# wgurecky/CORRLA_RS

Measured on AMD Instinct MI355X. Metric: RSVD GFLOP/s on 16k x 16k f32 rank-128, higher is better.
Workload: dtype f32

## Files before the change

### corrla_rs_amd/csrc/capi_impl.hpp

```cpp
#pragma once
#include <cstddef>
#include <cstdint>
#include <cstring>
#include <string>
#include <vector>

#include "../../include/corrla_rsvd.h"
#include "driver.hpp"

namespace corrla {

inline std::string& last_error_slot() {
  static thread_local std::string msg;
  return msg;
}

template <class F>
inline corrla_status guarded(F&& f) {
  try {
    f();
    return CORRLA_OK;
  } catch (const Error& e) {
    last_error_slot() = e.what();
    return (corrla_status)e.code;
// ... 158 lines not shown
}

template <class Dev, class T>
inline void finish_call(RsvdDriver<Dev, T>& drv, Dev& dev, Timings* tm_out, bool with_sketch_kernel_ms) {
  PhaseTimer fin;
  drv.phase(drv.tm.finalize_ms, fin);
  dev.phase_end();
  dev.end_call();
  dev.phase_resolve(&drv.tm.total_ms);
  drv.tm.n_collectives = dev.n_collectives;
  drv.tm.collective_bytes = dev.collective_bytes;
  if (with_sketch_kernel_ms) drv.tm.sketch_kernel_ms = dev.event_elapsed_ms(0, 1);
  if (tm_out) *tm_out = drv.tm;
}

template <class T>
struct RsvdCall {
  bool host_ptrs;
  int64_t m, rank, n_iter, n_oversamples;
  const corrla_opts* opts;
  T* u;
  int64_t ldu;
  T* s;
  T* vt;
  int64_t ldvt;
  Timings* tm_out;
  bool profile;
  bool sharded = false, sparse = false, fat = false, empty_shard = false;
  bool bf16 = false;
};
// ... 21 lines not shown
      },
      [&] {
        ta = stage();
        l = std::min<int64_t>(c.rank + c.n_oversamples, ta.nt);
        if (ro.omega && ro.omega_ld < ta.nt) throw Error(ST_EINVAL, "omega_ld < min(m, n)");
        u_in_place = !c.fat && !c.host_ptrs && !c.empty_shard;
        ut = u_in_place ? caller_skinny(c.u, ta.mt, k, c.ldu) : dev.template alloc_skinny<T>(ta.mt, k);
        vtall = dev.template alloc_skinny<T>(ta.nt, k);
        s_dev = dev.template alloc_scalar<T>((int)k);
      });
  RsvdDriver<Dev, T> drv(dev, c.profile);
  if (c.empty_shard) drv.m_local_override_ = 0;
  drv.random_svd_tall(ta, k, l, c.n_iter, ro, ut, s_dev, vtall, [&] {
    if (!c.fat) {
      if (!u_in_place && !c.empty_shard) dev.copy_out(ut, k, c.u, c.ldu, false, c.host_ptrs);
      dev.copy_out(vtall, k, c.vt, c.ldvt, true, c.host_ptrs);
    } else {
      dev.copy_out(vtall, k, c.u, c.ldu, false, c.host_ptrs);
      if (!c.empty_shard) dev.copy_out(ut, k, c.vt, c.ldvt, true, c.host_ptrs);
    }
    dev.copy_values_out(s_dev, k, c.s, c.host_ptrs);
  });
  finish_call(drv, dev, c.tm_out, true);
}

template <class Dev, class T>
inline void rsvd_entry(Dev& dev, bool host_ptrs, bool sharded, const T* a, int64_t m, int64_t n, int64_t rs, int64_t cs,
                       int64_t rank, int64_t n_iter, int64_t n_oversamples, const corrla_opts* opts, T* u, int64_t ldu,
                       T* s, T* vt, int64_t ldvt, Timings* tm_out, bool profile) {
  const bool shard_cols = sharded && opts && (opts->flags & CORRLA_SHARD_COLS) != 0;
  const bool empty_shard = sharded && m >= 0 && n >= 0 && (shard_cols ? (n == 0 && m >= 1) : (m == 0 && n >= 1));
  const int64_t short_side = shard_cols ? m : n;
  RsvdCall<T> c{host_ptrs, m, rank, n_iter, n_oversamples, opts, u, ldu, s, vt, ldvt, tm_out, profile};
  c.sharded = sharded;
  c.fat = sharded ? shard_cols : m < n;
  c.empty_shard = empty_shard;
// ... 104 lines not shown
    } else {
      dev.center_rows_cols(ta.mem.p, ta.mem.rows, ta.mem.cols, ta.mem.ld, mu.p, data_cols_along_mem_cols, cbuf, ldp);
    }
    tc.mem.p = cbuf;
    tc.mem.ld = ldp;
    tc.mem.cols_readable = ldp;
  }
  const int64_t k = c.rank;
  const int64_t l = std::min<int64_t>(c.rank + c.n_oversamples, tc.nt);
  if (ro.omega && ro.omega_ld < tc.nt) throw Error(ST_EINVAL, "omega_ld < min(m, n)");
  Skinny<T> ut = dev.template alloc_skinny<T>(tc.mt, k);
  Skinny<T> vtall = dev.template alloc_skinny<T>(tc.nt, k);
  T* s_dev = dev.template alloc_scalar<T>((int)k);
  if (tc.inv_sd_short || tc.inv_sd_tall) drv.set_scale_workspace(dev.template alloc_skinny<T>(c.n, l));
  drv.random_svd_tall(tc, k, l, c.n_iter, ro, ut, s_dev, vtall, [&] {
    dev.copy_out(fat ? ut : vtall, k, c.comps, c.ldc, true, c.host_ptrs);
    dev.copy_values_out(s_dev, k, c.s, c.host_ptrs);
    dev.copy_values_out(mu.p, c.n, c.means, c.host_ptrs);
    if (scales_out) dev.copy_values_out(sd.p, c.n, scales_out, c.host_ptrs);
  });
  finish_call(drv, dev, c.tm_out, false);
}

template <class Dev, class T>
inline void pca_entry(Dev& dev, bool host_ptrs, const T* x, int64_t m, int64_t n, int64_t rs, int64_t cs, int64_t rank,
                      int64_t n_iter, int64_t n_oversamples, const corrla_opts* opts, T* means, T* s, T* comps,
                      int64_t ldc, Timings* tm_out, bool profile, bool sharded = false) {
  PcaCall<T> c{host_ptrs, m, n, rank, n_iter, n_oversamples, opts, means, s, comps, ldc, tm_out, profile};
  c.sharded = sharded;
  pca_body(
      dev, c,
      [&] {
// ... 249 lines not shown
```

### corrla_rs_amd/csrc/core_svd_stage.hpp

```cpp
#pragma once
#include "core_svd_plan.hpp"
#include "hip_backend.hpp"

namespace corrla {

template <class T>
struct CoreSvdCall {
  const Skinny<T>& c;
  int64_t l, k;
  Skinny<T>&m1, &m2;
  T* s_dev;
  void* conv_status;
};

namespace core_svd_stage {

template <class T>
using RingEs = std::integer_sequence<int, 8, 12, 16, sizeof(T) == 4 ? 20 : 18>;
constexpr int kMaxNc = 9;

template <class T>
inline void set_lds_limits() {
  for_each_of(RingEs<T>{}, [](auto e) { lds_limit((const void*)k::jacobi_ring_w_kernel<T, decltype(e)::value, 8>, k::kLdsMaxBytes); });
  lds_limit((const void*)k::jacobi_block_round_kernel<T>, k::kLdsMaxBytes);
// ... 146 lines not shown
  kn.jmc_np = env_int("CORRLA_JMC_NP", kn.jmc_np);
  kn.jmc_sweeps_f32 = env_int("CORRLA_JMC_SWEEPS", kn.jmc_sweeps_f32);
  kn.jmc_sweeps_f64 = env_int("CORRLA_JMC_SWEEPS", kn.jmc_sweeps_f64);
  kn.jmc_force_v = env_int("CORRLA_JMC_FORCE_V", 0) != 0;
  kn.strict = env_int("CORRLA_JACOBI_STRICT", 0) != 0;
  kn.block_sweeps = env_int("CORRLA_JACOBI_SWEEPS", kn.block_sweeps);
  kn.ring_sweeps = env_int("CORRLA_JACOBI_SWEEPS", kn.ring_sweeps);
  kn.block_inner = env_int("CORRLA_JACOBI_INNER", kn.block_inner);
  return kn;
}

}

template <class T>
void HipDev::small_svd(const Skinny<T>& c, int64_t l, int64_t k, Skinny<T>& m1, Skinny<T>& m2, T* s_dev, void* conv_status) {
  if (conv_status) memset_zero(conv_status, sizeof(k::CholStatus));
  const CoreSvdCall<T> a{c, l, k, m1, m2, s_dev, conv_status};
  const CoreSvdPlan plan = core_svd_plan((int)sizeof(T), l, k, core_svd_stage::knobs_from_env(), svd_state_, conv_status != nullptr);
  switch (plan.family) {
    case CoreSvd::kMultiWg:
      core_svd_stage::multi_wg(*this, a, plan);
      return;
    case CoreSvd::kHost:
      small_svd_host(*this, c, l, k, m1, m2, s_dev);
      return;
    case CoreSvd::kBlock:
      core_svd_stage::finite_check(*this, a);
      core_svd_stage::block(*this, a, plan);
      return;
    case CoreSvd::kRing:
      core_svd_stage::finite_check(*this, a);
// ... 7 lines not shown
```

### corrla_rs_amd/csrc/driver.hpp

```cpp
#pragma once
#include <cstdio>
#include <chrono>
#include <cmath>
#include <cstdint>
#include <cstring>
#include <limits>
#include <stdexcept>
#include <string>
#include <functional>
#include <type_traits>
#include <vector>

#include "gemm_plan.hpp"
#include "small_linalg.hpp"

namespace corrla {

struct Error : std::runtime_error {
  int code;
  Error(int c, const std::string& m) : std::runtime_error(m), code(c) {}
};
enum { ST_OK = 0, ST_EINVAL = 1, ST_ENOMEM = 2, ST_EHIP = 3, ST_ECOMM = 4, ST_ENUMERIC = 5, ST_ENODEV = 6 };

inline int64_t round_up(int64_t x, int64_t a) { return (x + a - 1) / a * a; }
// ... 43 lines not shown

template <class D, class = void>
struct dev_has_spmm : std::false_type {};
template <class D>
struct dev_has_spmm<D, std::void_t<decltype(D::kHasSpmm)>> : std::true_type {};

template <class D, class = void>
struct dev_has_bf16in : std::false_type {};
template <class D>
struct dev_has_bf16in<D, std::void_t<decltype(D::kHasBf16In)>> : std::true_type {};

template <class D, class = void>
struct dev_has_colvar : std::false_type {};
template <class D>
struct dev_has_colvar<D, std::void_t<decltype(D::kHasColVar)>> : std::true_type {};

template <class T>
struct TallA {
  Big<T> mem;
  bool row_major = true;
  int64_t mt = 0, nt = 0;
  const T* mu_short = nullptr;
  const T* mu_tall = nullptr;
  const T* inv_sd_short = nullptr;
  const T* inv_sd_tall = nullptr;
  bool sparse = false;
  CsrView<T> csr, csr_t;
  bool bf16 = false;
  Big<uint16_t> mem16;
};
// ... 91 lines not shown
    else if (a.bf16)
      bf16_times(!a.row_major, a.mem16, x, y, scale_dev);
    else if (mixed_planes_ && dev.template mixed_fits<T>(!a.row_major, a.mem, x, y))
      dev.gemm_mixed(!a.row_major, a.mem, x, y, scale_dev, mixed_planes_), ++tm.n_mixed_products;
    else if (a.row_major)
      dev.gemm_nn(a.mem, x, y, scale_dev);
    else
      dev.gemm_tn(a.mem, x, y, scale_dev);
    if (a.mu_short || a.mu_tall) {
      T* v = dev.template alloc_scalar<T>((int)x.cols_alloc);
      dev.weighted_colsum(x, a.nt, a.mu_short, v);
      dev.rank1_sub(y, a.mt, a.mu_tall, v, scale_dev);
    }
    if (a.inv_sd_tall) scale_output(y, a.mt, a.inv_sd_tall);
  }
  void at_times(const TallA<T>& a, const Skinny<T>& y_in, Skinny<T>& z, const T* scale_dev, bool sharded) {
    const Skinny<T> y = a.inv_sd_tall ? scaled_input(y_in, a.mt, a.inv_sd_tall) : y_in;
    if (a.sparse)
      sparse_times(a.csr_t, y, z, scale_dev);
    else if (a.bf16)
      bf16_times(a.row_major, a.mem16, y, z, scale_dev);
    else if (mixed_planes_ && dev.template mixed_fits<T>(a.row_major, a.mem, y, z))
      dev.gemm_mixed(a.row_major, a.mem, y, z, scale_dev, mixed_planes_), ++tm.n_mixed_products;
    else if (a.row_major)
      dev.gemm_tn(a.mem, y, z, scale_dev);
    else
      dev.gemm_nn(a.mem, y, z, scale_dev);
    if (a.mu_short || a.mu_tall) {
      T* v = dev.template alloc_scalar<T>((int)y.cols_alloc);
      dev.weighted_colsum(y, a.mt, a.mu_tall, v);
      dev.rank1_sub(z, a.nt, a.mu_short, v, scale_dev);
// ... 436 lines not shown
      }
      a_times(a, z, y, kNone);
      i0 = nf;
    } else {
      dev.event_mark(0);
      a_times(a, om, y, kNone);
      dev.event_mark(1);
      phase(tm.sketch_ms, pt);
    }
    for (int64_t i = i0; i < n_iter; ++i) {
      if (i > 2) {
        phase(tm.power_ms, pt);
        orthonormalize(y, y2, o.sharded, true);
        phase(tm.qr_ms, pt);
      }
      at_times(a, y, z, kNone, o.sharded);
      dev.inv_norm(z, ss_dev, inv_dev);
      dev.scale_inplace(z, inv_dev);
      a_times(a, z, y, kNone);
    }
    phase(tm.power_ms, pt);
    int64_t r = orthonormalize(y, y2, o.sharded);
    phase(tm.qr_ms, pt);
    return r;
  }

  void random_svd_tall(const TallA<T>& a, int64_t k, int64_t l, int64_t n_iter, const RunOpts& o, Skinny<T>& u_tall,
                       T* s_dev, Skinny<T>& v_tall, const std::function<void()>& emit = {}) {
    qr_householder = o.qr_householder;
    m_local_ = m_local_override_ >= 0 ? m_local_override_ : a.mt;
    m_global_ = -1;
    hh_short_shards_ = -1;
    const bool hh = qr_householder;
    if (!hh && (dev.template device_chol_fits<T>(l) || dev.template device_chol_blocked_fits<T>(l))) {
      const Timings saved = tm;
      const auto mark = dev.arena_mark();
      bool on_device = true;
      for (int attempt = 0; attempt < 5 && on_device; ++attempt) {
        if (attempt > 0) dev.arena_rewind(mark);
// ... 100 lines not shown
    }
    return need[p.npass - 1] != 0 ? Verdict::kMorePasses : Verdict::kClean;
  }
  Verdict judge_core_svd(const Pending& p, const StatusRecord& r) {
    debug_record(p.record, "core SVD", r);
    if (r.fail == 0) dev.svd_sweeps_used((int)r.dev_i);
    if (r.fail == 1) return Verdict::kMoreSweeps;
    if (r.fail == 4) return Verdict::kNeedV;
    return r.fail == 0 ? Verdict::kClean : Verdict::kRepeatOnHost;
  }

  void random_svd_tall_body(const TallA<T>& a, int64_t k, int64_t l, int64_t n_iter, const RunOpts& o, Skinny<T>& u_tall,
                            T* s_dev, Skinny<T>& v_tall) {
    PhaseTimer total;
    const bool hh_tmp = qr_householder;
    Skinny<T> q = dev.template alloc_skinny_out<T>(a.mt, l);
    Skinny<T> q2 = hh_tmp ? dev.template alloc_skinny<T>(a.mt, l) : dev.template alloc_skinny_out<T>(a.mt, l);
    power_iter(a, l, n_iter, o, q, q2);
    PhaseTimer pt;
    Skinny<T> bt = dev.template alloc_skinny<T>(a.nt, l);
    mixed_planes_ = o.mixed_project ? o.mixed_planes : 0;
    at_times(a, q, bt, kNone, o.sharded);
    mixed_planes_ = 0;
    phase(tm.project_ms, pt);
    Skinny<T> qb = dev.template alloc_skinny<T>(a.nt, l);
    Skinny<T> qb2 = dev.template alloc_skinny<T>(a.nt, l);
    dev.copy_skinny(bt, qb);
    orthonormalize(qb, qb2, false);
    phase(tm.qr_ms, pt);
    Skinny<T> ct = dev.template alloc_skinny<T>(l, l);
    dev.gemm_nn(as_rowmajor_transposed(bt, l), qb, ct, kNone);
    if (o.poison_core) dev.poison_entry(ct, l / 2, l / 3, o.poison_core);
    Skinny<T> m1 = dev.template alloc_skinny<T>(l, k);
    Skinny<T> m2 = dev.template alloc_skinny<T>(l, k);
    void* svd_st = nullptr;
    if (att_.defer && att_.st_used + 1 <= att_.st_slots) {
      svd_st = status_record(att_.st_used);
      att_.pending.push_back(Pending::core_svd(att_.st_used));
      att_.st_used += 1;
    }
    dev.small_svd(ct, l, k, m2, m1, s_dev, svd_st);
    if (att_.defer) {
// ... 94 lines not shown
```

### corrla_rs_amd/csrc/hip_backend.hpp

```cpp
#pragma once
#include <hip/hip_runtime.h>
#include <rccl/rccl.h>

#include <cmath>
#include <cstdio>
#include <cstdlib>
#include <cstring>
#include <limits>
#include <random>
#include <string>
#include <type_traits>
#include <utility>
#include <vector>

#include "core_svd_plan.hpp"
#include "driver.hpp"
#include "hip_kernels.hpp"
#include "tsqr_kernels.hpp"
#include "jacobi_mc_kernels.hpp"
#include "ata_kernels.hpp"
#include "tall_kernels.hpp"
#include "mixed_kernels.hpp"
#include "bf16in_kernels.hpp"
#include "grad_kernels.hpp"
// ... 161 lines not shown
      *nranks_out = 0;
      return;
    }
    CORRLA_NCCL(ncclCommUserRank(comm, rank_out));
    CORRLA_NCCL(ncclCommCount(comm, nranks_out));
  }

  void begin_call() {
    CORRLA_HIP(hipSetDevice(device));
    events_set_[0] = events_set_[1] = events_set_[2] = false;
    n_collectives = 0;
    collective_bytes = 0;
    marks_.clear();
    ev_used_ = 0;
    phase_mark(nullptr);
    for (auto& c : chunks_) c.used = 0;
    sp_scratch_ = nullptr;
    sp_scratch_bytes_ = 0;
    for (auto& c : zchunks_) {
      c.zeroed = std::min<size_t>(c.used, (size_t)256 << 20);
      c.used = 0;
      if (c.zeroed) CORRLA_HIP(hipMemsetAsync(c.p, 0, c.zeroed, stream));
    }
  }
  void end_call() { sync(); }
  void sync() { CORRLA_HIP(hipStreamSynchronize(stream)); }

  void* alloc_bytes(size_t bytes) {
    bytes = (bytes + 255) / 256 * 256;
    if (bytes == 0) bytes = 256;
// ... 61 lines not shown
    s.cols = cols;
    s.ld = round_up(std::max<int64_t>(rows, 1), kLdPad);
    s.cols_alloc = col_blocking(cols).cols_alloc;
    const size_t bytes = (size_t)s.ld * (size_t)s.cols_alloc * sizeof(T);
    if (bytes < ((size_t)4 << 20)) {
      s.p = (T*)alloc_zeroed(bytes);
      return s;
    }
    s.p = (T*)alloc_bytes(bytes);
    if (s.ld > rows)
      CORRLA_HIP(hipMemset2DAsync(s.p + rows, (size_t)s.ld * sizeof(T), 0, (size_t)(s.ld - rows) * sizeof(T), (size_t)s.cols_alloc,
                                  stream));
    if (s.cols_alloc > cols) memset_zero(s.p + cols * s.ld, (size_t)(s.cols_alloc - cols) * s.ld * sizeof(T));
    return s;
  }
  double* alloc_f64(int n) {
    return (double*)alloc_zeroed(sizeof(double) * n);
  }
  template <class T>
  T* alloc_scalar(int n) {
    return (T*)alloc_zeroed(sizeof(T) * n);
  }

  void h2d_2d(void* dst, int64_t dpitch_e, const void* src, int64_t spitch_e, int64_t width_e, int64_t rows, size_t esz) {
    CORRLA_HIP(hipMemcpy2DAsync(dst, (size_t)dpitch_e * esz, src, (size_t)spitch_e * esz, (size_t)width_e * esz,
                                (size_t)rows, hipMemcpyHostToDevice, stream));
    sync();
  }
  template <class T>
  void h2d_2d(T* dst, int64_t dpitch_e, const T* src, int64_t spitch_e, int64_t width_e, int64_t rows) {
    h2d_2d((void*)dst, dpitch_e, (const void*)src, spitch_e, width_e, rows, sizeof(T));
  }

  template <class T>
  void gemm_nn(const Big<T>& r, const Skinny<T>& x, Skinny<T>& out, const T* scale_dev) {
    if (x.rows != r.cols) throw Error(ST_EINVAL, "gemm_nn: inner dimensions differ");
    launch_gemm<T>(false, r, x, out, scale_dev);
  }
  template <class T>
  void gemm_tn(const Big<T>& r, const Skinny<T>& x, Skinny<T>& out, const T* scale_dev) {
    if (x.rows != r.rows) throw Error(ST_EINVAL, "gemm_tn: inner dimensions differ");
    launch_gemm<T>(true, r, x, out, scale_dev);
  }

  static constexpr bool kHasSpmm = true;
  template <class T>
  void csr_plan(CsrView<T>& v, bool check_idx) {
    k::CsrCounts* cnt = (k::CsrCounts*)alloc_zeroed(sizeof(k::CsrCounts));
    const int64_t top = std::max(v.rows, v.nnz);
    const unsigned blocks = (unsigned)std::max<int64_t>(1, std::min<int64_t>((top + 255) / 256, (int64_t)num_cus * 16));
    hipLaunchKernelGGL(k::csr_validate_kernel, dim3(blocks), dim3(256), 0, stream, v.rp, v.ci, v.rows, v.cols, v.nnz, check_idx ? 1 : 0, cnt);
    CORRLA_HIP(hipGetLastError());
    k::CsrCounts h;
    read_bytes(cnt, sizeof(h), &h);
    if (h.bad) {
      std::string why;
      if (h.bad & 1) why += " row_ptr[0] != 0;";
// ... 585 lines not shown
  void householder_thin_q(Skinny<T>& y, Skinny<T>& tmp) {
    HhState<T> h = householder_up(y, tmp);
    householder_down(h, y, tmp);
  }
  template <class T>
  int householder_max_width() const {
    int w = 1;
    while (householder_fits<T>(w + 1)) ++w;
    return w;
  }
  int rank() const { return comm_rank; }

  template <class T>
  void small_svd(const Skinny<T>& c, int64_t l, int64_t k, Skinny<T>& m1, Skinny<T>& m2, T* s_dev, void* conv_status);
  template <class T>
  void copy_out(const Skinny<T>& src, int64_t ncols, T* dst, int64_t ldd, bool transpose, bool to_host) {
    const int64_t rows = src.rows;
    if (!to_host) {
      launch_copy_out(src.p, src.ld, rows, ncols, dst, ldd, transpose);
      return;
    }
    if (!transpose) {
      CORRLA_HIP(hipMemcpy2DAsync(dst, (size_t)ldd * sizeof(T), src.p, (size_t)src.ld * sizeof(T),
                                  (size_t)rows * sizeof(T), (size_t)ncols, hipMemcpyDeviceToHost, stream));
    } else {
      T* tmp = (T*)alloc_bytes((size_t)rows * ncols * sizeof(T));
      launch_copy_out(src.p, src.ld, rows, ncols, tmp, ncols, true);
      CORRLA_HIP(hipMemcpy2DAsync(dst, (size_t)ldd * sizeof(T), tmp, (size_t)ncols * sizeof(T),
                                  (size_t)ncols * sizeof(T), (size_t)rows, hipMemcpyDeviceToHost, stream));
    }
    sync();
  }
  template <class T>
  void pack_strided(const T* src, int64_t rows, int64_t cols, int64_t rs, int64_t cs, T* dst, int64_t ldd) {
    const int64_t tiles_c = (cols + 31) / 32, tiles_r = (rows + 31) / 32;
    if (tiles_c * tiles_r > 0x7fffffff) throw Error(ST_EINVAL, "problem too large for the launch grid");
    dim3 grid((unsigned)(tiles_c * tiles_r));
    hipLaunchKernelGGL((k::pack_strided_kernel<T>), grid, dim3(256), 0, stream, src, rows, cols, rs, cs, dst, ldd, tiles_c);
    CORRLA_HIP(hipGetLastError());
  }

  template <class T>
  void weighted_colsum(const Skinny<T>& x, int64_t rows, const T* w, T* v) {
    const int ncols = (int)x.cols_alloc;
    const int nblk = (int)std::max<int64_t>(1, std::min<int64_t>(64, (rows + 4095) / 4096));
    double* partial = (double*)alloc_bytes(sizeof(double) * (size_t)nblk * (size_t)ncols);
// ... 226 lines not shown
  hipEvent_t events_[3] = {nullptr, nullptr, nullptr};
  bool events_set_[3] = {false, false, false};
  struct PhaseMark {
    hipEvent_t ev;
    double* slot;
  };
  std::vector<hipEvent_t> ev_pool_;
  size_t ev_used_ = 0;
  std::vector<PhaseMark> marks_;
  static constexpr size_t kPinnedBytes = (size_t)8 << 20;
  int gemm_debug_flags_ = 0;
  GemmKnobs gemm_knobs_;
  uint64_t entropy_ = 0, calls_ = 0, calls_sharded_ = 0;
  bool no_device_chol_ = false;
  const int* run_if_ = nullptr;
  bool phase_events_ = true;
  bool robust_qr_ = true;
  int robust_passes_ = 2;
  CoreSvdState svd_state_;

  static void check_grid(const dim3& g) {
    if (g.y > 65535u || g.z > 65535u) throw Error(ST_EINVAL, "problem too large for the launch grid");
  }

  static void set_lds_limits() {
    constexpr size_t kMax = k::kLdsMaxBytes;
    set_lds_limits_typed<float>();
    set_lds_limits_typed<double>();
    core_svd_stage::set_lds_limits<float>();
    core_svd_stage::set_lds_limits<double>();
// ... 104 lines not shown
  void launch_general(bool tn, const GemmPlan& p, dim3 grid, dim3 block, int lds, const k::GemmArgs<T>& a) {
    with_nt<2>(p.mw, [&](auto mw) {
      with_nt<8, 4>(p.nw, [&](auto nw) {
        constexpr int MW = decltype(mw)::value, NW = decltype(nw)::value;
        if constexpr (NW == 4 || (NW == 8 && MW == 1 && std::is_same<T, double>::value)) {
          if (tn)
            hipLaunchKernelGGL((k::gemm_tn_kernel<T, MW, NT, NW>), grid, block, lds, stream, a);
          else
            hipLaunchKernelGGL((k::gemm_nn_kernel<T, MW, NT, false, NW>), grid, block, lds, stream, a);
        }
      });
    });
  }

  template <class T>
  void launch_gemm(bool tn, const Big<T>& r, const Skinny<T>& x, Skinny<T>& out, const T* scale_dev) {
    const GemmPlan p = plan_gemm(tn, r, x, out, 0);
    const GemmLaunch& L0 = p.launch[0];
    T* slab = p.reduce.kind != SlabReduce::none ? (T*)alloc_bytes(p.slab_bytes) : nullptr;
    if (p.family == GemmFamily::tall_apply) {
      const k::TallApplyArgs<T> g{r.p, r.cols, r.ld, (int)r.rows, x.p, x.ld, (int)x.cols, out.p, out.ld, (int)p.out_cols,
                                  scale_dev, p.vec_store, run_if_};
      with_nt<sizeof(T) == 4 ? 6 : 4>(L0.nt, [&](auto kt) {
        constexpr int K = decltype(kt)::value;
        hipLaunchKernelGGL((k::tall_apply_kernel<T, K, K>), dim3(L0.grid[0]), dim3(p.block), L0.lds, stream, g);
      });
    } else if (p.family == GemmFamily::tall_gram) {
      const k::TallGramArgs<T> g{x.p, r.cols, x.ld, (int)out.rows, slab, p.slab_stride, out.ld, p.rows_per_group,
                                 (const T*)zero_page_, run_if_};
      with_nt<sizeof(T) == 4 ? 6 : 4>(L0.nt, [&](auto nct) {
        hipLaunchKernelGGL((k::tall_gram_kernel<T, decltype(nct)::value>), dim3(L0.grid[0]), dim3(p.block), L0.lds, stream, g);
// ... 7 lines not shown
                       p.vec_store, p.rotate, p.outer_blocks, 0};
      for (int i = 0; i < p.nlaunch; ++i) {
        const GemmLaunch& L = p.launch[i];
        const dim3 grid(L.grid[0], L.grid[1], L.grid[2]), block(p.block);
        a.col_base = L.col_base;
        a.xcd_remap = L.xcd_remap;
        if (p.family == GemmFamily::gram_alias)
          with_nt<8>(L.nt, [&](auto nt) {
            hipLaunchKernelGGL((k::gemm_nn_kernel<T, 2, decltype(nt)::value, true>), grid, block, L.lds, stream, a);
          });
        else
          with_nt<kMaxColTiles>(L.nt, [&](auto nt) { launch_general<T, decltype(nt)::value>(tn, p, grid, block, L.lds, a); });
      }
    }
    CORRLA_HIP(hipGetLastError());
    slab_reduce<T>(p.reduce, slab, p.slab_stride, out.p, out.ld, scale_dev, run_if_);
  }

  template <class T>
  void launch_copy_out(const T* src, int64_t lds_, int64_t rows, int64_t cols, T* dst, int64_t ldd, bool transpose) {
    const int64_t tiles_c = (cols + 31) / 32, tiles_r = (rows + 31) / 32;
    if (tiles_c * tiles_r > 0x7fffffff) throw Error(ST_EINVAL, "problem too large for the launch grid");
    dim3 grid((unsigned)(tiles_c * tiles_r));
    hipLaunchKernelGGL((k::copy_out_kernel<T>), grid, dim3(256), 0, stream, src, lds_, rows, cols, dst, ldd,
                       transpose ? 1 : 0, tiles_c);
    CORRLA_HIP(hipGetLastError());
  }
};

}
```

### corrla_rs_amd/csrc/hip_kernels.hpp

```cpp
#pragma once
#include <hip/hip_runtime.h>

#include <limits>
#include <stdint.h>

#include <type_traits>

#include "gemm_plan.hpp"

namespace corrla {
namespace k {

typedef float f32x4 __attribute__((ext_vector_type(4)));
typedef double f64x4 __attribute__((ext_vector_type(4)));
typedef double f64x2 __attribute__((ext_vector_type(2)));

#ifndef CORRLA_F32_BIG_IS_A
#define CORRLA_F32_BIG_IS_A true
#endif
template <class T>
struct MT;
template <>
struct MT<float> {
  typedef f32x4 acc_t;
// ... 672 lines not shown
    const double v = (double)y[i];
    s += v * v;
  }
  for (int off = 32; off > 0; off >>= 1) s += __shfl_down(s, off, 64);
  __shared__ double ws[4];
  if ((threadIdx.x & 63) == 0) ws[threadIdx.x >> 6] = s;
  __syncthreads();
  if (threadIdx.x == 0) partial[blockIdx.x] = ws[0] + ws[1] + ws[2] + ws[3];
}
__global__ void sum_partials_kernel(const double* partial, int n, double* out) {
  double s = 0.0;
  for (int i = threadIdx.x; i < n; i += 64) s += partial[i];
  for (int off = 32; off > 0; off >>= 1) s += __shfl_down(s, off, 64);
  if (threadIdx.x == 0) *out = s;
}
template <class T>
__global__ void sum_partials_rsqrt_kernel(const double* partial, int n, double* ss_out, T* inv_out) {
  double s = 0.0;
  for (int i = threadIdx.x; i < n; i += 64) s += partial[i];
  for (int off = 32; off > 0; off >>= 1) s += __shfl_down(s, off, 64);
  if (threadIdx.x == 0) {
    *ss_out = s;
    *inv_out = (T)(s > 0.0 ? 1.0 / sqrt(s) : 0.0);
  }
}
template <class T>
__global__ void rsqrt_scalar_kernel(const double* ss, T* out) {
  const double v = *ss;
  *out = (T)(v > 0.0 ? 1.0 / sqrt(v) : 0.0);
}
template <class T>
__global__ void sub_kernel(T* y, const T* __restrict__ p, int64_t n) {
  for (int64_t i = (int64_t)blockIdx.x * blockDim.x + threadIdx.x; i < n; i += (int64_t)gridDim.x * blockDim.x) y[i] -= p[i];
}
template <class T>
__global__ void scale_kernel(T* y, int64_t n, const T* scale) {
  const T sc = *scale;
  for (int64_t i = (int64_t)blockIdx.x * blockDim.x + threadIdx.x; i < n; i += (int64_t)gridDim.x * blockDim.x)
// ... 1191 lines not shown
  const int tx = threadIdx.x & 31, ty = threadIdx.x >> 5;
  const bool col_fast = cs <= rs;
  for (int q = ty; q < 32; q += 8) {
    const int64_t r = col_fast ? r0 + q : r0 + tx;
    const int64_t c = col_fast ? c0 + tx : c0 + q;
    if (r < rows && c < cols) tile[r - r0][c - c0] = src[r * rs + c * cs];
  }
  __syncthreads();
  for (int q = ty; q < 32; q += 8) {
    const int64_t r = r0 + q, c = c0 + tx;
    if (r < rows && c < cols) dst[r * ldd + c] = tile[q][tx];
  }
}
template <class T>
__global__ void copy_out_kernel(const T* src, int64_t lds_, int64_t rows, int64_t cols, T* dst, int64_t ldd, int transpose,
                                int64_t tiles_c) {
  __shared__ T tile[32][33];
  const int64_t r0 = ((int64_t)blockIdx.x / tiles_c) * 32, c0 = ((int64_t)blockIdx.x % tiles_c) * 32;
  const int tx = threadIdx.x & 31, ty = threadIdx.x >> 5;
  if (!transpose) {
    for (int q = ty; q < 32; q += 8) {
      const int64_t r = r0 + tx, c = c0 + q;
      if (r < rows && c < cols) dst[c * ldd + r] = src[c * lds_ + r];
    }
    return;
  }
  for (int q = ty; q < 32; q += 8) {
    const int64_t r = r0 + tx, c = c0 + q;
    if (r < rows && c < cols) tile[q][tx] = src[c * lds_ + r];
  }
  __syncthreads();
  for (int q = ty; q < 32; q += 8) {
// ... 8 lines not shown
```

Measured before the change: 93540.

## Fuse RSVD tail ops into slab reduce, copy-out and padding kernels

Adds several tail fusions. The split-K slab reduction now also writes a second copy of the output (replacing a separate copy_skinny) and emits per-block sum-of-squares partials, so normalisation takes one scale kernel instead of a norm-then-scale pair. Singular values ride along in the copy-out kernel, the conv-status memset is skipped, and the two output Q buffers are padded by one zeroing kernel. The aim is fewer small kernel launches and fewer passes over the skinny matrices, at the cost of extra code paths gated on plan family and the CORRLA_TAIL_UNFUSED env var.

```diff
diff --git a/corrla_rs_amd/csrc/capi_impl.hpp b/corrla_rs_amd/csrc/capi_impl.hpp
--- a/corrla_rs_amd/csrc/capi_impl.hpp
+++ b/corrla_rs_amd/csrc/capi_impl.hpp
@@ -196,6 +196,17 @@
   if (tm_out) *tm_out = drv.tm;
 }
 
+template <class Dev, class T>
+inline void copy_out_with_s(Dev& dev, const Skinny<T>& src, int64_t k, T* dst, int64_t ldd, bool transpose, bool host_ptrs,
+                            const T* s_dev, T* s_out) {
+  if constexpr (dev_has_tail_fusions<Dev>::value) {
+    dev.copy_out_with_values(src, k, dst, ldd, transpose, host_ptrs, s_dev, s_out, k);
+  } else {
+    dev.copy_out(src, k, dst, ldd, transpose, host_ptrs);
+    dev.copy_values_out(s_dev, k, s_out, host_ptrs);
+  }
+}
+
 template <class T>
 struct RsvdCall {
   bool host_ptrs;
@@ -247,12 +258,11 @@
   drv.random_svd_tall(ta, k, l, c.n_iter, ro, ut, s_dev, vtall, [&] {
     if (!c.fat) {
       if (!u_in_place && !c.empty_shard) dev.copy_out(ut, k, c.u, c.ldu, false, c.host_ptrs);
-      dev.copy_out(vtall, k, c.vt, c.ldvt, true, c.host_ptrs);
+      copy_out_with_s(dev, vtall, k, c.vt, c.ldvt, true, c.host_ptrs, s_dev, c.s);
     } else {
-      dev.copy_out(vtall, k, c.u, c.ldu, false, c.host_ptrs);
       if (!c.empty_shard) dev.copy_out(ut, k, c.vt, c.ldvt, true, c.host_ptrs);
+      copy_out_with_s(dev, vtall, k, c.u, c.ldu, false, c.host_ptrs, s_dev, c.s);
     }
-    dev.copy_values_out(s_dev, k, c.s, c.host_ptrs);
   });
   finish_call(drv, dev, c.tm_out, true);
 }
@@ -387,8 +397,7 @@
   T* s_dev = dev.template alloc_scalar<T>((int)k);
   if (tc.inv_sd_short || tc.inv_sd_tall) drv.set_scale_workspace(dev.template alloc_skinny<T>(c.n, l));
   drv.random_svd_tall(tc, k, l, c.n_iter, ro, ut, s_dev, vtall, [&] {
-    dev.copy_out(fat ? ut : vtall, k, c.comps, c.ldc, true, c.host_ptrs);
-    dev.copy_values_out(s_dev, k, c.s, c.host_ptrs);
+    copy_out_with_s(dev, fat ? ut : vtall, k, c.comps, c.ldc, true, c.host_ptrs, s_dev, c.s);
     dev.copy_values_out(mu.p, c.n, c.means, c.host_ptrs);
     if (scales_out) dev.copy_values_out(sd.p, c.n, scales_out, c.host_ptrs);
   });
diff --git a/corrla_rs_amd/csrc/core_svd_stage.hpp b/corrla_rs_amd/csrc/core_svd_stage.hpp
--- a/corrla_rs_amd/csrc/core_svd_stage.hpp
+++ b/corrla_rs_amd/csrc/core_svd_stage.hpp
@@ -184,7 +184,7 @@
 
 template <class T>
 void HipDev::small_svd(const Skinny<T>& c, int64_t l, int64_t k, Skinny<T>& m1, Skinny<T>& m2, T* s_dev, void* conv_status) {
-  if (conv_status) memset_zero(conv_status, sizeof(k::CholStatus));
+  if (conv_status && tail_unfused_) memset_zero(conv_status, sizeof(k::CholStatus));
   const CoreSvdCall<T> a{c, l, k, m1, m2, s_dev, conv_status};
   const CoreSvdPlan plan = core_svd_plan((int)sizeof(T), l, k, core_svd_stage::knobs_from_env(), svd_state_, conv_status != nullptr);
   switch (plan.family) {
diff --git a/corrla_rs_amd/csrc/driver.hpp b/corrla_rs_amd/csrc/driver.hpp
--- a/corrla_rs_amd/csrc/driver.hpp
+++ b/corrla_rs_amd/csrc/driver.hpp
@@ -81,6 +81,28 @@
 struct dev_has_colvar : std::false_type {};
 template <class D>
 struct dev_has_colvar<D, std::void_t<decltype(D::kHasColVar)>> : std::true_type {};
+
+template <class D, class = void>
+struct dev_has_tail_fusions : std::false_type {};
+template <class D>
+struct dev_has_tail_fusions<D, std::void_t<decltype(D::kHasTailFusions)>> : std::true_type {};
+
+template <class T>
+struct ProductTaps {
+  T* copy_to = nullptr;
+  bool want_sumsq = false;
+  bool copied = false;
+  const double* partial = nullptr;
+  int nparts = 0;
+};
+struct TapContext {
+  bool tail_fused = false;
+  bool sparse = false, bf16 = false, centred = false, standardised = false, sharded = false;
+  int mixed_planes = 0;
+};
+inline bool product_taps_apply(const TapContext& c) {
+  return c.tail_fused && !c.sparse && !c.bf16 && c.mixed_planes == 0 && !c.centred && !c.standardised && !c.sharded;
+}
 
 template <class T>
 struct TallA {
@@ -202,7 +224,26 @@
     }
     if (a.inv_sd_tall) scale_output(y, a.mt, a.inv_sd_tall);
   }
-  void at_times(const TallA<T>& a, const Skinny<T>& y_in, Skinny<T>& z, const T* scale_dev, bool sharded) {
+  bool tail_fused() const {
+    if constexpr (dev_has_tail_fusions<Dev>::value)
+      return dev.tail_fused();
+    else
+      return false;
+  }
+  bool taps_apply(const TallA<T>& a, bool sharded) const {
+    TapContext c;
+    c.tail_fused = tail_fused();
+    c.sparse = a.sparse, c.bf16 = a.bf16, c.mixed_planes = mixed_planes_, c.sharded = sharded;
+    c.centred = a.mu_short || a.mu_tall, c.standardised = a.inv_sd_short || a.inv_sd_tall;
+    return product_taps_apply(c);
+  }
+  void at_times(const TallA<T>& a, const Skinny<T>& y_in, Skinny<T>& z, const T* scale_dev, bool sharded, ProductTaps<T>* taps = nullptr) {
+    if (taps && taps_apply(a, sharded)) {
+      if constexpr (dev_has_tail_fusions<Dev>::value) {
+        dev.gemm_tapped(a.row_major, a.mem, y_in, z, scale_dev, *taps);
+        return;
+      }
+    }
     const Skinny<T> y = a.inv_sd_tall ? scaled_input(y_in, a.mt, a.inv_sd_tall) : y_in;
     if (a.sparse)
       sparse_times(a.csr_t, y, z, scale_dev);
@@ -669,15 +710,29 @@
         orthonormalize(y, y2, o.sharded, true);
         phase(tm.qr_ms, pt);
       }
-      at_times(a, y, z, kNone, o.sharded);
-      dev.inv_norm(z, ss_dev, inv_dev);
-      dev.scale_inplace(z, inv_dev);
+      ProductTaps<T> taps;
+      taps.want_sumsq = true;
+      at_times(a, y, z, kNone, o.sharded, &taps);
+      if (!normalize_from_taps(z, taps, ss_dev, inv_dev)) {
+        dev.inv_norm(z, ss_dev, inv_dev);
+        dev.scale_inplace(z, inv_dev);
+      }
       a_times(a, z, y, kNone);
     }
     phase(tm.power_ms, pt);
     int64_t r = orthonormalize(y, y2, o.sharded);
     phase(tm.qr_ms, pt);
     return r;
+  }
+
+  bool normalize_from_taps(Skinny<T>& z, const ProductTaps<T>& taps, double* ss_dev, T* inv_dev) {
+    if constexpr (dev_has_tail_fusions<Dev>::value) {
+      if (taps.nparts > 0) {
+        dev.scale_by_partials(z, taps, ss_dev, inv_dev);
+        return true;
+      }
+    }
+    return false;
   }
 
   void random_svd_tall(const TallA<T>& a, int64_t k, int64_t l, int64_t n_iter, const RunOpts& o, Skinny<T>& u_tall,
@@ -808,18 +863,26 @@
                             T* s_dev, Skinny<T>& v_tall) {
     PhaseTimer total;
     const bool hh_tmp = qr_householder;
-    Skinny<T> q = dev.template alloc_skinny_out<T>(a.mt, l);
-    Skinny<T> q2 = hh_tmp ? dev.template alloc_skinny<T>(a.mt, l) : dev.template alloc_skinny_out<T>(a.mt, l);
+    Skinny<T> q, q2;
+    if constexpr (dev_has_tail_fusions<Dev>::value) {
+      if (!hh_tmp) dev.template alloc_skinny_out2<T>(a.mt, l, q, q2);
+    }
+    if (!q.p) {
+      q = dev.template alloc_skinny_out<T>(a.mt, l);
+      q2 = hh_tmp ? dev.template alloc_skinny<T>(a.mt, l) : dev.template alloc_skinny_out<T>(a.mt, l);
+    }
     power_iter(a, l, n_iter, o, q, q2);
     PhaseTimer pt;
     Skinny<T> bt = dev.template alloc_skinny<T>(a.nt, l);
+    Skinny<T> qb = dev.template alloc_skinny<T>(a.nt, l);
+    ProductTaps<T> bt_taps;
+    bt_taps.copy_to = qb.p;
     mixed_planes_ = o.mixed_project ? o.mixed_planes : 0;
-    at_times(a, q, bt, kNone, o.sharded);
+    at_times(a, q, bt, kNone, o.sharded, &bt_taps);
     mixed_planes_ = 0;
     phase(tm.project_ms, pt);
-    Skinny<T> qb = dev.template alloc_skinny<T>(a.nt, l);
     Skinny<T> qb2 = dev.template alloc_skinny<T>(a.nt, l);
-    dev.copy_skinny(bt, qb);
+    if (!bt_taps.copied) dev.copy_skinny(bt, qb);
     orthonormalize(qb, qb2, false);
     phase(tm.qr_ms, pt);
     Skinny<T> ct = dev.template alloc_skinny<T>(l, l);
diff --git a/corrla_rs_amd/csrc/hip_backend.hpp b/corrla_rs_amd/csrc/hip_backend.hpp
--- a/corrla_rs_amd/csrc/hip_backend.hpp
+++ b/corrla_rs_amd/csrc/hip_backend.hpp
@@ -199,6 +199,7 @@
     marks_.clear();
     ev_used_ = 0;
     phase_mark(nullptr);
+    tail_unfused_ = env_int("CORRLA_TAIL_UNFUSED", 0) != 0;
     for (auto& c : chunks_) c.used = 0;
     sp_scratch_ = nullptr;
     sp_scratch_bytes_ = 0;
@@ -290,6 +291,25 @@
     if (s.cols_alloc > cols) memset_zero(s.p + cols * s.ld, (size_t)(s.cols_alloc - cols) * s.ld * sizeof(T));
     return s;
   }
+  template <class T>
+  void alloc_skinny_out2(int64_t rows, int64_t cols, Skinny<T>& a, Skinny<T>& b) {
+    const int64_t ld = round_up(std::max<int64_t>(rows, 1), kLdPad), cols_alloc = col_blocking(cols).cols_alloc;
+    const size_t bytes = (size_t)ld * (size_t)cols_alloc * sizeof(T);
+    const int64_t n = (ld - rows) * cols + (cols_alloc - cols) * ld;
+    if (tail_unfused_ || bytes < ((size_t)4 << 20) || (size_t)n * sizeof(T) > ((size_t)4 << 20)) {
+      a = alloc_skinny_out<T>(rows, cols);
+      b = alloc_skinny_out<T>(rows, cols);
+      return;
+    }
+    a.rows = rows, a.cols = cols, a.ld = ld, a.cols_alloc = cols_alloc;
+    b = a;
+    a.p = (T*)alloc_bytes(bytes);
+    b.p = (T*)alloc_bytes(bytes);
+    if (n == 0) return;
+    const dim3 grid((unsigned)std::min<int64_t>(1024, (n + 255) / 256), 2);
+    hipLaunchKernelGGL((k::zero_padding2_kernel<T>), grid, dim3(256), 0, stream, a.p, b.p, ld, rows, cols, cols_alloc);
+    CORRLA_HIP(hipGetLastError());
+  }
   double* alloc_f64(int n) {
     return (double*)alloc_zeroed(sizeof(double) * n);
   }
@@ -317,6 +337,21 @@
   void gemm_tn(const Big<T>& r, const Skinny<T>& x, Skinny<T>& out, const T* scale_dev) {
     if (x.rows != r.rows) throw Error(ST_EINVAL, "gemm_tn: inner dimensions differ");
     launch_gemm<T>(true, r, x, out, scale_dev);
+  }
+  static constexpr bool kHasTailFusions = true;
+  bool tail_fused() const { return !tail_unfused_; }
+  template <class T>
+  void gemm_tapped(bool tn, const Big<T>& r, const Skinny<T>& x, Skinny<T>& out, const T* scale_dev, ProductTaps<T>& taps) {
+    if (x.rows != (tn ? r.rows : r.cols)) throw Error(ST_EINVAL, "gemm_tapped: inner dimensions differ");
+    launch_gemm<T>(tn, r, x, out, scale_dev, &taps);
+  }
+  template <class T>
+  void scale_by_partials(Skinny<T>& y, const ProductTaps<T>& taps, double* ss_dev, T* inv_dev) {
+    const int64_t n = y.ld * y.cols_alloc;
+    const int blocks = (int)std::min<int64_t>(4096, std::max<int64_t>(1, (n + 256 * k::kScalePre - 1) / (256 * k::kScalePre)));
+    hipLaunchKernelGGL((k::scale_by_partials_kernel<T>), dim3(blocks), dim3(256), 0, stream, y.p, n, taps.partial, taps.nparts, ss_dev,
+                       inv_dev);
+    CORRLA_HIP(hipGetLastError());
   }
 
   static constexpr bool kHasSpmm = true;
@@ -932,12 +967,14 @@
   template <class T>
   void small_svd(const Skinny<T>& c, int64_t l, int64_t k, Skinny<T>& m1, Skinny<T>& m2, T* s_dev, void* conv_status);
   template <class T>
-  void copy_out(const Skinny<T>& src, int64_t ncols, T* dst, int64_t ldd, bool transpose, bool to_host) {
+  void copy_out(const Skinny<T>& src, int64_t ncols, T* dst, int64_t ldd, bool transpose, bool to_host, const T* vals_src = nullptr,
+                T* vals_dst = nullptr, int64_t nvals = 0) {
     const int64_t rows = src.rows;
     if (!to_host) {
-      launch_copy_out(src.p, src.ld, rows, ncols, dst, ldd, transpose);
+      launch_copy_out(src.p, src.ld, rows, ncols, dst, ldd, transpose, vals_src, vals_dst, nvals);
       return;
     }
+    if (nvals > 0) throw Error(ST_EINVAL, "internal: values ride on a device-to-device copy_out only");
     if (!transpose) {
       CORRLA_HIP(hipMemcpy2DAsync(dst, (size_t)ldd * sizeof(T), src.p, (size_t)src.ld * sizeof(T),
                                   (size_t)rows * sizeof(T), (size_t)ncols, hipMemcpyDeviceToHost, stream));
@@ -948,6 +985,17 @@
                                   (size_t)ncols * sizeof(T), (size_t)rows, hipMemcpyDeviceToHost, stream));
     }
     sync();
+  }
+  template <class T>
+  void copy_out_with_values(const Skinny<T>& src, int64_t ncols, T* dst, int64_t ldd, bool transpose, bool to_host,
+                            const T* vals_dev, T* vals_dst, int64_t nvals) {
+    const bool ride = nvals > 0 && !to_host && !tail_unfused_;
+    if (ride) {
+      copy_out(src, ncols, dst, ldd, transpose, false, vals_dev, vals_dst, nvals);
+    } else {
+      copy_out(src, ncols, dst, ldd, transpose, to_host);
+      copy_values_out(vals_dev, nvals, vals_dst, to_host);
+    }
   }
   template <class T>
   void pack_strided(const T* src, int64_t rows, int64_t cols, int64_t rs, int64_t cs, T* dst, int64_t ldd) {
@@ -1204,6 +1252,7 @@
   uint64_t entropy_ = 0, calls_ = 0, calls_sharded_ = 0;
   bool no_device_chol_ = false;
   const int* run_if_ = nullptr;
+  bool tail_unfused_ = false;
   bool phase_events_ = true;
   bool robust_qr_ = true;
   int robust_passes_ = 2;
@@ -1338,7 +1387,7 @@
   }
 
   template <class T>
-  void launch_gemm(bool tn, const Big<T>& r, const Skinny<T>& x, Skinny<T>& out, const T* scale_dev) {
+  void launch_gemm(bool tn, const Big<T>& r, const Skinny<T>& x, Skinny<T>& out, const T* scale_dev, ProductTaps<T>* taps = nullptr) {
     const GemmPlan p = plan_gemm(tn, r, x, out, 0);
     const GemmLaunch& L0 = p.launch[0];
     T* slab = p.reduce.kind != SlabReduce::none ? (T*)alloc_bytes(p.slab_bytes) : nullptr;
@@ -1376,16 +1425,37 @@
       }
     }
     CORRLA_HIP(hipGetLastError());
-    slab_reduce<T>(p.reduce, slab, p.slab_stride, out.p, out.ld, scale_dev, run_if_);
-  }
-
-  template <class T>
-  void launch_copy_out(const T* src, int64_t lds_, int64_t rows, int64_t cols, T* dst, int64_t ldd, bool transpose) {
+    if (taps && !tail_unfused_ && p.reduce.kind != SlabReduce::none && p.family == GemmFamily::general && !out.external && !run_if_)
+      slab_reduce_tapped<T>(p.reduce, slab, p.slab_stride, out, scale_dev, *taps);
+    else
+      slab_reduce<T>(p.reduce, slab, p.slab_stride, out.p, out.ld, scale_dev, run_if_);
+  }
+  template <class T>
+  void slab_reduce_tapped(const SlabReducePlan& rp, const T* slab, int64_t stride, Skinny<T>& out, const T* scale, ProductTaps<T>& taps) {
+    const int64_t n = out.ld * out.cols_alloc;
+    const int blocks = (int)std::min<int64_t>(1024, std::max<int64_t>(1, (n + 255) / 256));
+    const int64_t step = (int64_t)blocks * 256;
+    double* partial = taps.want_sumsq ? (double*)alloc_bytes(sizeof(double) * blocks) : nullptr;
+    if (rp.kind == SlabReduce::deep)
+      hipLaunchKernelGGL((k::slab_reduce_tap_kernel<T, true>), dim3(blocks), dim3(256), 0, stream, slab, stride, rp.slabs, out.p,
+                         taps.copy_to, out.ld, rp.rows, rp.cols, n, step / out.ld, step % out.ld, scale, partial);
+    else
+      hipLaunchKernelGGL((k::slab_reduce_tap_kernel<T, false>), dim3(blocks), dim3(256), 0, stream, slab, stride, rp.slabs, out.p,
+                         taps.copy_to, out.ld, rp.rows, rp.cols, n, step / out.ld, step % out.ld, scale, partial);
+    CORRLA_HIP(hipGetLastError());
+    taps.copied = taps.copy_to != nullptr;
+    taps.partial = partial;
+    taps.nparts = partial ? blocks : 0;
+  }
+
+  template <class T>
+  void launch_copy_out(const T* src, int64_t lds_, int64_t rows, int64_t cols, T* dst, int64_t ldd, bool transpose,
+                       const T* vals_src = nullptr, T* vals_dst = nullptr, int64_t nvals = 0) {
     const int64_t tiles_c = (cols + 31) / 32, tiles_r = (rows + 31) / 32;
     if (tiles_c * tiles_r > 0x7fffffff) throw Error(ST_EINVAL, "problem too large for the launch grid");
     dim3 grid((unsigned)(tiles_c * tiles_r));
     hipLaunchKernelGGL((k::copy_out_kernel<T>), grid, dim3(256), 0, stream, src, lds_, rows, cols, dst, ldd,
-                       transpose ? 1 : 0, tiles_c);
+                       transpose ? 1 : 0, tiles_c, vals_src, vals_dst, nvals);
     CORRLA_HIP(hipGetLastError());
   }
 };
diff --git a/corrla_rs_amd/csrc/hip_kernels.hpp b/corrla_rs_amd/csrc/hip_kernels.hpp
--- a/corrla_rs_amd/csrc/hip_kernels.hpp
+++ b/corrla_rs_amd/csrc/hip_kernels.hpp
@@ -710,14 +710,162 @@
   for (int off = 32; off > 0; off >>= 1) s += __shfl_down(s, off, 64);
   if (threadIdx.x == 0) *out = s;
 }
+__device__ __forceinline__ double sum_partials_wave(const double* partial, int n, int lane) {
+  double v[16];
+#pragma unroll
+  for (int u = 0; u < 16; ++u) v[u] = partial[min(lane + 64 * u, n - 1)];
+  double s = 0.0;
+#pragma unroll
+  for (int u = 0; u < 16; ++u)
+    if (lane + 64 * u < n) s += v[u];
+  for (int i = lane + 1024; i < n; i += 64) s += partial[i];
+  for (int off = 32; off > 0; off >>= 1) s += __shfl_down(s, off, 64);
+  return s;
+}
+template <class T>
+__device__ __forceinline__ T inv_sqrt_or_zero(double s) {
+  return (T)(s > 0.0 ? 1.0 / sqrt(s) : 0.0);
+}
 template <class T>
 __global__ void sum_partials_rsqrt_kernel(const double* partial, int n, double* ss_out, T* inv_out) {
-  double s = 0.0;
-  for (int i = threadIdx.x; i < n; i += 64) s += partial[i];
-  for (int off = 32; off > 0; off >>= 1) s += __shfl_down(s, off, 64);
+  const double s = sum_partials_wave(partial, n, (int)threadIdx.x);
   if (threadIdx.x == 0) {
     *ss_out = s;
-    *inv_out = (T)(s > 0.0 ? 1.0 / sqrt(s) : 0.0);
+    *inv_out = inv_sqrt_or_zero<T>(s);
+  }
+}
+template <class T>
+__device__ __forceinline__ T slab_sum_plain(const T* __restrict__ src, int64_t slab_stride, int nsplit) {
+  T s = 0;
+  for (int z = 0; z < nsplit; ++z) s += src[(int64_t)z * slab_stride];
+  return s;
+}
+template <class T>
+__device__ __forceinline__ T slab_sum_deep(const T* __restrict__ src, int64_t slab_stride, int nsplit) {
+  const int per = (nsplit + 3) / 4;
+  T part[4];
+#pragma unroll
+  for (int zg = 0; zg < 4; ++zg) {
+    const int z0 = zg * per, z1 = min(nsplit, z0 + per);
+    T s0 = 0, s1 = 0, s2 = 0, s3 = 0;
+    int z = z0;
+    for (; z + 3 < z1; z += 4) {
+      s0 += src[(int64_t)z * slab_stride];
+      s1 += src[(int64_t)(z + 1) * slab_stride];
+      s2 += src[(int64_t)(z + 2) * slab_stride];
+      s3 += src[(int64_t)(z + 3) * slab_stride];
+    }
+    for (; z < z1; ++z) s0 += src[(int64_t)z * slab_stride];
+    part[zg] = (s0 + s1) + (s2 + s3);
+  }
+  return (part[0] + part[1]) + (part[2] + part[3]);
+}
+template <class T, bool DEEP>
+__global__ __launch_bounds__(256) void slab_reduce_tap_kernel(const T* __restrict__ slab, int64_t slab_stride, int nsplit,
+                                                              T* __restrict__ out, T* __restrict__ out2, int64_t ld, int64_t limit,
+                                                              int64_t ncols, int64_t n, int64_t step_q, int64_t step_r, const T* scale,
+                                                              double* partial) {
+  constexpr int U = DEEP ? 2 : 8;
+  const int64_t stride = (int64_t)gridDim.x * blockDim.x;
+  const int64_t i0 = (int64_t)blockIdx.x * blockDim.x + threadIdx.x;
+  int64_t col = 0, row = i0;
+  if (ld <= i0) {
+    col = (int64_t)((uint32_t)i0 / (uint32_t)ld);
+    row = i0 - col * ld;
+  }
+  const T sc = scale ? *scale : (T)1;
+  double s = 0.0;
+  for (int64_t base = i0; base < n; base += U * stride) {
+    int64_t idx[U];
+    bool in[U];
+    T x[U];
+#pragma unroll
+    for (int u = 0; u < U; ++u) {
+      const int64_t i = base + u * stride;
+      in[u] = i < n && row < limit && col < ncols;
+      idx[u] = in[u] ? i : 0;
+      col += step_q;
+      row += step_r;
+      if (row >= ld) {
+        row -= ld;
+        ++col;
+      }
+    }
+    if constexpr (DEEP) {
+#pragma unroll
+      for (int u = 0; u < U; ++u) x[u] = slab_sum_deep(slab + idx[u], slab_stride, nsplit);
+    } else {
+#pragma unroll
+      for (int u = 0; u < U; ++u) x[u] = 0;
+      for (int z = 0; z < nsplit; ++z) {
+        const T* src = slab + (int64_t)z * slab_stride;
+#pragma unroll
+        for (int u = 0; u < U; ++u) x[u] += src[idx[u]];
+      }
+    }
+#pragma unroll
+    for (int u = 0; u < U; ++u) {
+      double v = 0.0;
+      if (in[u]) {
+        T y = x[u];
+        if (scale) y *= sc;
+        out[idx[u]] = y;
+        if (out2) out2[idx[u]] = y;
+        v = (double)y;
+      }
+      s += v * v;
+    }
+  }
+  if (!partial) return;
+  for (int off = 32; off > 0; off >>= 1) s += __shfl_down(s, off, 64);
+  __shared__ double ws[4];
+  if ((threadIdx.x & 63) == 0) ws[threadIdx.x >> 6] = s;
+  __syncthreads();
+  if (threadIdx.x == 0) partial[blockIdx.x] = ws[0] + ws[1] + ws[2] + ws[3];
+}
+constexpr int kScalePre = 4;
+template <class T>
+__global__ __launch_bounds__(256) void scale_by_partials_kernel(T* y, int64_t n, const double* partial, int nparts, double* ss_out,
+                                                                T* inv_out) {
+  __shared__ T sc_sh;
+  const int64_t stride = (int64_t)gridDim.x * blockDim.x;
+  const int64_t i0 = (int64_t)blockIdx.x * blockDim.x + threadIdx.x;
+  T pre[kScalePre];
+#pragma unroll
+  for (int u = 0; u < kScalePre; ++u) {
+    const int64_t i = i0 + u * stride;
+    pre[u] = y[i < n ? i : 0];
+  }
+  if (threadIdx.x < 64) {
+    const double s = sum_partials_wave(partial, nparts, (int)threadIdx.x);
+    if (threadIdx.x == 0) {
+      sc_sh = inv_sqrt_or_zero<T>(s);
+      if (blockIdx.x == 0) {
+        *ss_out = s;
+        *inv_out = sc_sh;
+      }
+    }
+  }
+  __syncthreads();
+  const T sc = sc_sh;
+#pragma unroll
+  for (int u = 0; u < kScalePre; ++u) {
+    const int64_t i = i0 + u * stride;
+    if (i < n) y[i] = pre[u] * sc;
+  }
+  for (int64_t i = i0 + kScalePre * stride; i < n; i += stride) y[i] *= sc;
+}
+template <class T>
+__global__ void zero_padding2_kernel(T* a, T* b, int64_t ld, int64_t rows, int64_t cols, int64_t cols_alloc) {
+  T* p = blockIdx.y == 0 ? a : b;
+  const int64_t pr = ld - rows, n_rows = pr * cols, n_cols = (cols_alloc - cols) * ld;
+  for (int64_t i = (int64_t)blockIdx.x * blockDim.x + threadIdx.x; i < n_rows + n_cols; i += (int64_t)gridDim.x * blockDim.x) {
+    if (i < n_rows) {
+      const int64_t c = i / pr;
+      p[c * ld + rows + (i - c * pr)] = (T)0;
+    } else {
+      p[cols * ld + (i - n_rows)] = (T)0;
+    }
   }
 }
 template <class T>
@@ -1939,8 +2087,10 @@
 }
 template <class T>
 __global__ void copy_out_kernel(const T* src, int64_t lds_, int64_t rows, int64_t cols, T* dst, int64_t ldd, int transpose,
-                                int64_t tiles_c) {
+                                int64_t tiles_c, const T* vals_src = nullptr, T* vals_dst = nullptr, int64_t nvals = 0) {
   __shared__ T tile[32][33];
+  if (vals_dst && blockIdx.x == 0)
+    for (int64_t i = threadIdx.x; i < nvals; i += blockDim.x) vals_dst[i] = vals_src[i];
   const int64_t r0 = ((int64_t)blockIdx.x / tiles_c) * 32, c0 = ((int64_t)blockIdx.x % tiles_c) * 32;
   const int tx = threadIdx.x & 31, ty = threadIdx.x >> 5;
   if (!transpose) {
```

After: 91820. -1.8%, worse.
